# NTV-UIT/MARLLB

Measured on AMD Instinct MI355X. Metric: env-steps/sec (whole node), 4-server LB env, batch 4k→512k at 1/2/4/8 MI355X, higher is better.
Workload: dtype fp32/int32 (f64 reward); 1 GPU; LB env random-policy rollout, 4 servers (BASELINE configs[1] rollout at the north-star batch); assign_policy=sed, envs_per_gpu=65536, servers=4, global_batch=65536, autoreset=True, autoreset_mode=same_step, parallelism=env-shard x1, dyn_mapping=auto

## Files before the change

### marllb_amd/csrc/lbsim_api.hip

```cpp
#include <hip/hip_runtime.h>

#include <cxxabi.h>

#include <algorithm>
#include <cmath>
#include <cstdarg>
#include <cstdio>
#include <cstdlib>
#include <cstring>
#include <string>
#include <vector>

#include "../../include/lbsim.h"
#include "lbsim_internal.h"
#include "lbsim_fused.h"
#include "lbsim_nets.h"
#include "lbsim_stateless.h"
#include "lbsim_vpp.h"

using namespace lbk;

namespace {
constexpr int kLogMax = 8;
thread_local const void* g_log_fn[kLogMax];
// ... 450 lines not shown
    for (int i = 0; i < g_log_n; ++i) v.emplace_back(g_log_cls[i], g_log_fn[i]);
    h->launched_lost[which] = g_log_lost;
    g_log_n = 0;
    g_log_lost = 0;
    g_log_class = -1;
  }
};

std::string short_kernel_name(const char* raw) {
  std::string s = raw ? raw : "?";
  int st = 0;
  if (char* d = abi::__cxa_demangle(s.c_str(), nullptr, nullptr, &st)) {
    if (st == 0) s = d;
    free(d);
  }
  int depth = 0;
  for (size_t i = 0; i < s.size(); ++i) {
    if (s[i] == '<') ++depth;
    else if (s[i] == '>') --depth;
    else if (s[i] == '(' && depth == 0 && s.compare(i, 21, "(anonymous namespace)") != 0) {
      s.resize(i);
      break;
    }
  }
  for (const char* pre : {"void ", "lbk::", "(anonymous namespace)::"}) {
    for (size_t at; (at = s.find(pre)) != std::string::npos;) s.erase(at, strlen(pre));
  }
  return s;
}

LaunchCtx ctx(const lbsim_t* h) { return LaunchCtx{h->plan, h->st, h->prm, h->flow}; }

StepPlan plan_of(const lbsim_t* h) {
  static const Overrides ov = Overrides::from_env();
  const SimParams& p = h->prm;
  PlanInput in{};
  in.B = h->B, in.S = h->S, in.Q = p.Q, in.policy = p.policy;
  in.trace = p.trace != 0, in.fail = p.fail_thr != 0u, in.leak = p.leak != 0;
  in.split = p.split != 0, in.res_vpp = p.res_vpp != 0, in.dur_plane = dur_plane(p);
  in.next_reset = p.next_reset != 0;
  in.flow_stats = h->flow.hist != nullptr;
  in.dyn_mapping = h->cfg.dyn_mapping, in.step_kernel = h->cfg.step_kernel, in.simds = h->simds;
  return make_plan(in, ov);
}

int launch_dynamics(lbsim_t* h, const void* action, int dtype, int32_t* assign,
                    const uint8_t* mask, int mode, hipStream_t stream) {
  ProfScope ps(h, stream, mode == kModeStep ? 0 : 2);
  if (mode == kModeStep && h->plan.nr)
    launch_dynamics_step_nr(ctx(h), action, dtype, assign, mask, stream);
  else if (mode == kModeStep)
    launch_dynamics_step(ctx(h), action, dtype, assign, mask, stream);
  else
    launch_dynamics_reset(ctx(h), action, dtype, assign, mask, stream);
  return launch_check(h, "dynamics_kernel");
}

bool facade_bad(const lbsim_t* h, const lbsim_step_outputs_t* out) {
  if (out->agent_obs == nullptr && out->state == nullptr) return false;
  return out->num_agents < 1 || out->servers_per_agent < 1 ||
         (int64_t)out->num_agents * out->servers_per_agent != h->S;
}

ObsOutputs obs_outputs(const lbsim_step_outputs_t* out, bool reset) {
  ObsOutputs o{};
  o.obs = out->obs;
  o.raw_obs = out->raw_obs;
  if (!reset) {
    o.reward = out->reward;
    o.done = out->done;
    o.ep_len = out->episode_length;
    o.ep_ret = out->episode_return;
    o.done_word = out->done_word;
    o.done_value = out->done_value;
  }
  o.agent_obs = out->agent_obs;
  o.state = out->state;
  o.num_agents = out->num_agents;
  o.servers_per_agent = out->servers_per_agent;
  return o;
}

int launch_observe(lbsim_t* h, const ObsOutputs& o, const uint8_t* mask, int mode,
                   hipStream_t stream) {
  ProfScope ps(h, stream, mode == kModeStep ? 1 : 3);
  if (mode == kModeStep) launch_observe_step(ctx(h), o, mask, stream);
  else launch_observe_reset(ctx(h), o, mask, stream);
  return launch_check(h, "observe_kernel");
}


int round16(int x) { return (x + 15) / 16 * 16; }

int fused_mt(int dflt) {
  static const int forced = env_int("LBSIM_FUSED_MT", 0);
  return (forced == 1 || forced == 2 || forced == 4) ? forced : dflt;
}

}

extern "C" {

const char* lbsim_version(void) { return "lbsim 0.1.0 (gfx950, HIP)"; }
int lbsim_abi_version(void) { return LBSIM_ABI_VERSION; }

int lbsim_config_default(lbsim_config_t* c) {
  if (c == nullptr) return LBSIM_EINVAL;
  memset(c, 0, sizeof(*c));
  c->num_envs = 1;
  c->num_servers = 4;
  c->env_id_offset = 0;
  c->seed = 0;
  c->action_type = LBSIM_ACTION_DISCRETE;
  c->num_discrete = 3;
  c->discrete_weights[0] = 1.0f;
  c->discrete_weights[1] = 1.5f;
  c->discrete_weights[2] = 2.0f;
  c->min_weight = 0.1f;
  c->max_weight = 10.0f;
  c->reward_metric = LBSIM_METRIC_JAIN;
  c->reward_field = 10;
  c->step_interval = 0.25f;
  c->max_steps = 10000;
  c->normalize_obs = 0;
  c->assign_policy = LBSIM_POLICY_SED;
  c->arrival_source = LBSIM_ARRIVAL_POISSON;
  c->arrival_rate = 400.0f;
  for (int s = 0; s < LBSIM_MAX_SERVERS; ++s) c->server_rate[s] = 125.0f;
  c->decay_factor = 0.9f;
  c->queue_capacity = 32;
  c->warmup_steps = 8;
  c->lost_fin_prob = 0.0f;
  c->flow_timeout_s = 40.0f;
  c->flow_buckets = 1024;
  c->fail_prob = 0.0f;
  c->recover_prob = 0.1f;
  c->duration_mode = LBSIM_DURATION_AGE;
  c->lost_fin_pending = 256;
  c->reservoir_mode = LBSIM_RESERVOIR_ALGR;
  return LBSIM_OK;
}

int lbsim_config_validate(const lbsim_config_t* cfg, char* msg, size_t msg_len) {
  return validate(cfg, msg, msg_len);
}

int lbsim_create(const lbsim_config_t* cfg, int device, lbsim_t** out) {
  if (out == nullptr) return fail(nullptr, LBSIM_EINVAL, "out is NULL");
  *out = nullptr;
  char msg[256] = {0};
  if (validate(cfg, msg, sizeof(msg)) != LBSIM_OK) return fail(nullptr, LBSIM_EINVAL, "%s", msg);
  int ndev = 0;
  if (hipGetDeviceCount(&ndev) != hipSuccess || ndev == 0)
    return fail(nullptr, LBSIM_EDEVICE, "no HIP device available");
  if (device < 0 || device >= ndev)
    return fail(nullptr, LBSIM_EINVAL, "device %d out of range [0, %d)", device, ndev);
  DeviceGuard g(device);
  if (!g.ok) return fail(nullptr, LBSIM_EDEVICE, "hipSetDevice(%d) failed", device);

  lbsim_t* h = new lbsim_t();
  h->cfg = *cfg;
  h->device = device;
  int cus = 0;
  if (hipDeviceGetAttribute(&cus, hipDeviceAttributeMultiprocessorCount, device) != hipSuccess ||
      cus < 1)
    cus = 256;
  h->simds = 4 * cus;
  h->B = cfg->num_envs;
  h->S = cfg->num_servers;
  h->Q = cfg->queue_capacity;
  h->initialised = false;
  memset(&h->st, 0, sizeof(h->st));
  derive_params(*cfg, h->prm);
  h->plan = plan_of(h);
  for (Section& sec : sections(h)) {
    void* p = nullptr;
    if (hipMalloc(&p, sec.bytes) != hipSuccess) {
      lbsim_destroy(h);
      return fail(nullptr, LBSIM_ENOMEM, "hipMalloc(%zu) failed", sec.bytes);
    }
    h->allocs.push_back(p);
    *sec.ptr = p;
    if (hipMemset(p, 0, sec.bytes) != hipSuccess) {
      lbsim_destroy(h);
      return fail(nullptr, LBSIM_EDEVICE, "hipMemset failed");
    }
  }
  if (cfg->normalize_obs) {
    const size_t n = (size_t)h->B * h->S * NF;
    hipLaunchKernelGGL(init_norm_std, dim3((unsigned)((n + 255) / 256)), dim3(256), 0, nullptr,
                       h->st.norm_std, n);
  }
  if (hipDeviceSynchronize() != hipSuccess) {
    lbsim_destroy(h);
    return fail(nullptr, LBSIM_EDEVICE, "device init failed");
  }
  *out = h;
  return LBSIM_OK;
}

int lbsim_destroy(lbsim_t* h) {
  if (h == nullptr) return LBSIM_OK;
  {
    DeviceGuard g(h->device);
    for (void* p : h->allocs) (void)hipFree(p);
    if (h->trace_buf) (void)hipFree(h->trace_buf);
    if (h->stats_buf) (void)hipFree(h->stats_buf);
    if (h->rates_buf) (void)hipFree(h->rates_buf);
    if (h->flow_buf) (void)hipFree(h->flow_buf);
    for (hipEvent_t e : h->prof.ev) (void)hipEventDestroy(e);
  }
  delete h;
  return LBSIM_OK;
}

const char* lbsim_last_error(const lbsim_t* h) {
  return h ? h->err.c_str() : g_create_err.c_str();
}

int lbsim_dynamics_kernel(const lbsim_t* h) {
  if (h == nullptr) return -1;
  return h->plan.dyn.kernel;
}

int lbsim_seed(lbsim_t* h, uint64_t seed) {
  if (h == nullptr) return LBSIM_EINVAL;
  DeviceGuard g(h->device);
  h->cfg.seed = seed;
  h->prm.key0 = (uint32_t)(seed & 0xFFFFFFFFull);
  h->prm.key1 = (uint32_t)(seed >> 32);
  if (hipMemset(h->st.episode, 0, (size_t)h->B * 4) != hipSuccess)
    return fail(h, LBSIM_EDEVICE, "hipMemset failed");
  return LBSIM_OK;
}

int lbsim_reset(lbsim_t* h, const uint8_t* env_mask, float* obs_out, void* stream) {
  lbsim_step_outputs_t o;
  memset(&o, 0, sizeof(o));
  o.obs = obs_out;
  return lbsim_reset_ex(h, env_mask, &o, stream);
}

int lbsim_reset_ex(lbsim_t* h, const uint8_t* env_mask, const lbsim_step_outputs_t* out,
                   void* stream) {
  if (h == nullptr) return LBSIM_EINVAL;
  if (out == nullptr || out->obs == nullptr) return fail(h, LBSIM_EINVAL, "obs_out is NULL");
  if (facade_bad(h, out)) return fail(h, LBSIM_EINVAL, "agent_obs / state need num_agents * "
                                                       "servers_per_agent == num_servers");
  if (h->prm.trace && h->prm.trace_rows == 0)
    return fail(h, LBSIM_EINVAL, "arrival_source TRACE: call lbsim_set_trace before lbsim_reset");
  DeviceGuard g(h->device);
  LaunchLog log(h, 1);
  const hipStream_t s = (hipStream_t)stream;
  h->reset_seen = true;
  int rc = launch_dynamics(h, nullptr, 0, nullptr, env_mask, kModeReset, s);
  if (rc != LBSIM_OK) return rc;
  const ObsOutputs o = obs_outputs(out, true);
  rc = launch_observe(h, o, env_mask, kModeReset, s);
  if (rc != LBSIM_OK) return rc;
  if (env_mask == nullptr) h->initialised = true;
  return LBSIM_OK;
}

int lbsim_step(lbsim_t* h, const void* action, int action_dtype, float* obs_out,
               float* reward_out, uint8_t* done_out, int32_t* assign_count_out, void* stream) {
  lbsim_step_outputs_t o;
  memset(&o, 0, sizeof(o));
  o.obs = obs_out;
  o.reward = reward_out;
  o.done = done_out;
  o.assign_count = assign_count_out;
  return lbsim_step_ex(h, action, action_dtype, &o, stream);
}

size_t lbsim_config_size(void) { return sizeof(lbsim_config_t); }
size_t lbsim_step_outputs_size(void) { return sizeof(lbsim_step_outputs_t); }

int lbsim_step_ex(lbsim_t* h, const void* action, int action_dtype,
                  const lbsim_step_outputs_t* out, void* stream) {
  if (h == nullptr) return LBSIM_EINVAL;
  if (!h->initialised) return fail(h, LBSIM_EINVAL, "call lbsim_reset before lbsim_step");
  if (out == nullptr || action == nullptr || out->obs == nullptr || out->reward == nullptr ||
      out->done == nullptr)
    return fail(h, LBSIM_EINVAL, "action/obs/reward/done buffers must be non-NULL");
  if (h->cfg.action_type == LBSIM_ACTION_DISCRETE) {
    if (action_dtype != LBSIM_DTYPE_I32 && action_dtype != LBSIM_DTYPE_I64)
      return fail(h, LBSIM_EINVAL, "discrete actions must be int32 or int64");
  } else if (action_dtype != LBSIM_DTYPE_F32) {
    return fail(h, LBSIM_EINVAL, "continuous actions must be float32");
  }
  if (facade_bad(h, out)) return fail(h, LBSIM_EINVAL, "agent_obs / state need num_agents * "
                                                       "servers_per_agent == num_servers");
  if (out->done_word != nullptr && h->B != 1)
    return fail(h, LBSIM_EINVAL, "done_word needs a one-env handle (num_envs = 1)");
  DeviceGuard g(h->device);
  LaunchLog log(h, 0);
  const hipStream_t s = (hipStream_t)stream;
  const ObsOutputs o = obs_outputs(out, false);
  if (h->plan.form == kStepWave) {
    ProfScope ps(h, s, 4);
    launch_step_wave(ctx(h), action, action_dtype, out->assign_count, o, s);
    return launch_check(h, "step_wave_kernel");
  }
  if (h->plan.form == kStepGroupFused) {
    ProfScope ps(h, s, 4);
    launch_fused_step(ctx(h), action, action_dtype, out->assign_count, o, s);
    return launch_check(h, "fused_step_kernel");
  }
  h->prof.chain = true;
  int rc = launch_dynamics(h, action, action_dtype, out->assign_count, nullptr, kModeStep, s);
  h->prof.chain = false;
  if (rc != LBSIM_OK) {
    h->prof.chain_ev = -1;
    return rc;
  }
  return launch_observe(h, o, nullptr, kModeStep, s);
}

int lbsim_step_stats(lbsim_t* h, int64_t* stats_out) {
  if (h == nullptr || stats_out == nullptr) return LBSIM_EINVAL;
  DeviceGuard g(h->device);
  if (h->stats_buf == nullptr && hipMalloc(&h->stats_buf, 16) != hipSuccess) {
    h->stats_buf = nullptr;
    return fail(h, LBSIM_ENOMEM, "hipMalloc(16) failed");
  }
  const int64_t n = (int64_t)h->B * h->S;
  unsigned long long host[2] = {0, 0};
  if (hipDeviceSynchronize() != hipSuccess || hipMemset(h->stats_buf, 0, 16) != hipSuccess)
    return fail(h, LBSIM_EDEVICE, "sync / memset failed");
  const int64_t blocks = std::min<int64_t>((n + 255) / 256, 4096);
  hipLaunchKernelGGL(step_stats_kernel, dim3((unsigned)blocks), dim3(256), 0, nullptr, h->st.chg,
                     h->st.hc, n, h->stats_buf);
  if (hipMemcpy(host, h->stats_buf, 16, hipMemcpyDeviceToHost) != hipSuccess)
    return fail(h, LBSIM_EDEVICE, "step_stats_kernel failed");
  stats_out[0] = (int64_t)host[0];
  stats_out[1] = (int64_t)host[1];
  return LBSIM_OK;
}

int lbsim_episode_stats(lbsim_t* h, int32_t* length_out, double* return_out, void* stream) {
  if (h == nullptr) return LBSIM_EINVAL;
  DeviceGuard g(h->device);
  hipLaunchKernelGGL(copy_episode_stats, dim3((unsigned)((h->B + 255) / 256)), dim3(256), 0,
                     (hipStream_t)stream, h->st.ep_step, h->st.ep_return, length_out, return_out,
                     h->B);
  return launch_check(h, "copy_episode_stats");
}

int lbsim_reward(const lbsim_config_t* cfg, const float* obs, int64_t n, float* reward_out,
                 void* stream) {
  if (cfg == nullptr || obs == nullptr || reward_out == nullptr || n < 0) return LBSIM_EINVAL;
  if (cfg->num_servers < 1 || cfg->num_servers > LBSIM_MAX_SERVERS) return LBSIM_EINVAL;
  if (cfg->reward_metric < 0 || cfg->reward_metric > 8) return LBSIM_EINVAL;
  if (n == 0) return LBSIM_OK;
  hipLaunchKernelGGL(reward_kernel, dim3((unsigned)((n + 255) / 256)), dim3(256), 0,
                     (hipStream_t)stream, obs, n, cfg->num_servers, cfg->reward_metric,
                     cfg->reward_field, reward_out);
  return hipGetLastError() == hipSuccess ? LBSIM_OK : LBSIM_EDEVICE;
}

int lbsim_set_trace(lbsim_t* h, const uint32_t* gap_us, const float* work, int64_t rows,
                    void* stream) {
  if (h == nullptr) return LBSIM_EINVAL;
  if (!h->prm.trace) return fail(h, LBSIM_EINVAL, "lbsim_set_trace needs arrival_source TRACE");
  if (gap_us == nullptr || work == nullptr || rows < 1 || rows > (int64_t)0x7FFFFFFF)
    return fail(h, LBSIM_EINVAL, "trace: need device gap_us/work and 1 <= rows < 2^31");
  DeviceGuard g(h->device);
  const hipStream_t s = (hipStream_t)stream;
  if (hipStreamSynchronize(s) != hipSuccess) return fail(h, LBSIM_EDEVICE, "stream sync failed");
  if (h->trace_buf) {
    (void)hipFree(h->trace_buf);
    h->trace_buf = nullptr;
    h->prm.trace_rows = 0;
  }
  const size_t n = (size_t)rows;
  if (hipMalloc(&h->trace_buf, n * 8) != hipSuccess) {
    h->trace_buf = nullptr;
    return fail(h, LBSIM_ENOMEM, "hipMalloc(%zu) failed", n * 8);
  }
  uint32_t* g_dev = (uint32_t*)h->trace_buf;
  float* w_dev = (float*)(g_dev + n);
  if (hipMemcpyAsync(g_dev, gap_us, n * 4, hipMemcpyDeviceToDevice, s) != hipSuccess ||
      hipMemcpyAsync(w_dev, work, n * 4, hipMemcpyDeviceToDevice, s) != hipSuccess ||
      hipStreamSynchronize(s) != hipSuccess)
    return fail(h, LBSIM_EDEVICE, "trace copy failed");
  h->st.trace_gap = g_dev;
  h->st.trace_work = w_dev;
  h->prm.trace_rows = (uint32_t)rows;
  return LBSIM_OK;
}

int lbsim_set_env_rates(lbsim_t* h, const float* arrival_rate, const float* server_rate,
                        void* stream) {
  if (h == nullptr) return LBSIM_EINVAL;
  if (arrival_rate != nullptr && h->prm.lf_thr != 0u)
    return fail(h, LBSIM_ENOTSUP, "per-env arrival rates on a lost-FIN handle (lost_fin_prob > 0): "
                                  "the bucket-wait mean and the 32-bit guess bound depend on the "
                                  "arrival rate (per-env server rates are allowed)");
  if (arrival_rate != nullptr && h->prm.trace)
    return fail(h, LBSIM_ENOTSUP, "per-env arrival rates on a TRACE handle: the trace sets the "
                                  "arrival rate (per-env server rates are allowed)");
  if (arrival_rate == nullptr && server_rate == nullptr) return LBSIM_OK;
  DeviceGuard g(h->device);
  const hipStream_t s = (hipStream_t)stream;
  int rc = env_rates_ensure(h, s);
  if (rc != LBSIM_OK) return rc;
  const size_t B = (size_t)h->B, BS = B * h->S;
  const EnvRates live = env_rates_live(h), stg = env_rates_staging(h);
  uint32_t* const bad = env_rates_bad(h);
  if (hipMemsetAsync(bad, 0, sizeof(uint32_t), s) != hipSuccess)
    return fail(h, LBSIM_EDEVICE, "per-env rates: hipMemsetAsync failed");
  hipLaunchKernelGGL(env_rates_kernel, dim3((unsigned)((BS + 255) / 256)), dim3(256), 0, s,
                     arrival_rate, (int64_t)1, server_rate, (int64_t)h->S, h->B, h->S, stg, bad);
  rc = launch_check(h, "env_rates_kernel");
  if (rc != LBSIM_OK) return rc;
  uint32_t nbad = 0;
  if (hipMemcpyAsync(&nbad, bad, sizeof(nbad), hipMemcpyDeviceToHost, s) != hipSuccess ||
      hipStreamSynchronize(s) != hipSuccess)
    return fail(h, LBSIM_EDEVICE, "per-env rates: conversion failed");
  if (nbad != 0u)
    return fail(h, LBSIM_EINVAL, "per-env rates: %u value(s) out of range (arrival_rate must be in "
                                 "[0.1, 1e6] flows/s, server_rate in [1, 1e7]; NaN rejected)", nbad);
  bool ok = true;
  if (arrival_rate != nullptr) {
    ok &= hipMemcpyAsync(live.arrival, stg.arrival, B * 4, hipMemcpyDeviceToDevice, s) == hipSuccess;
    ok &= hipMemcpyAsync(live.gap, stg.gap, B * 4, hipMemcpyDeviceToDevice, s) == hipSuccess;
  }
  if (server_rate != nullptr) {
    ok &= hipMemcpyAsync(live.server, stg.server, BS * 4, hipMemcpyDeviceToDevice, s) == hipSuccess;
    ok &= hipMemcpyAsync(live.scale, stg.scale, BS * 4, hipMemcpyDeviceToDevice, s) == hipSuccess;
  }
  if (!ok) return fail(h, LBSIM_EDEVICE, "per-env rates: device copy failed");
  h->st.env_gap = live.gap;
  h->st.env_scale = live.scale;
  return LBSIM_OK;
}

int lbsim_clear_env_rates(lbsim_t* h) {
  if (h == nullptr) return LBSIM_EINVAL;
  h->st.env_gap = nullptr;
  h->st.env_scale = nullptr;
  if (h->rates_buf == nullptr) return LBSIM_OK;
  DeviceGuard g(h->device);
  if (hipDeviceSynchronize() != hipSuccess) return fail(h, LBSIM_EDEVICE, "sync failed");
  env_rates_fill_defaults(h, nullptr);
  const int rc = launch_check(h, "env_rates_kernel");
  if (rc != LBSIM_OK) return rc;
  if (hipDeviceSynchronize() != hipSuccess) return fail(h, LBSIM_EDEVICE, "sync failed");
  return LBSIM_OK;
}

int lbsim_get_env_rates(lbsim_t* h, float* arrival_rate_out, float* server_rate_out,
                        void* stream) {
  if (h == nullptr) return LBSIM_EINVAL;
  if (arrival_rate_out == nullptr && server_rate_out == nullptr) return LBSIM_OK;
  DeviceGuard g(h->device);
  const hipStream_t s = (hipStream_t)stream;
  const int rc = env_rates_ensure(h, s);
  if (rc != LBSIM_OK) return rc;
  const size_t B = (size_t)h->B, BS = B * h->S;
  const EnvRates live = env_rates_live(h);
  bool ok = true;
  if (arrival_rate_out != nullptr)
    ok &= hipMemcpyAsync(arrival_rate_out, live.arrival, B * 4, hipMemcpyDeviceToDevice, s) == hipSuccess;
  if (server_rate_out != nullptr)
    ok &= hipMemcpyAsync(server_rate_out, live.server, BS * 4, hipMemcpyDeviceToDevice, s) == hipSuccess;
  return ok ? LBSIM_OK : fail(h, LBSIM_EDEVICE, "per-env rates: device copy failed");
}

int lbsim_flow_stats_enable(lbsim_t* h) {
  if (h == nullptr) return LBSIM_EINVAL;
  if (h->flow_buf != nullptr) return LBSIM_OK;
  if (h->reset_seen)
    return fail(h, LBSIM_EINVAL, "lbsim_flow_stats_enable must precede the handle's first "
                                 "lbsim_reset (the statistics change which kernels it launches)");
  DeviceGuard g(h->device);
  const size_t BS = (size_t)h->B * h->S, bytes = flow_stats_bytes(BS);
  void* p = nullptr;
  if (hipMalloc(&p, bytes) != hipSuccess) return fail(h, LBSIM_ENOMEM, "hipMalloc(%zu) failed", bytes);
  if (hipMemset(p, 0, bytes) != hipSuccess || hipDeviceSynchronize() != hipSuccess) {
    (void)hipFree(p);
    return fail(h, LBSIM_EDEVICE, "flow statistics: hipMemset failed");
  }
  h->flow_buf = p;
  h->flow.sum = (unsigned long long*)p;
  h->flow.hist = (uint32_t*)(h->flow.sum + BS);
  h->flow.count = h->flow.hist + BS * kFlowBins;
  h->flow.max_us = h->flow.count + BS;
  h->plan = plan_of(h);
  return LBSIM_OK;
}

int lbsim_flow_stats_get(lbsim_t* h, uint32_t* count, uint64_t* sum_us, uint32_t* max_us,
                         uint32_t* hist, void* stream) {
  if (h == nullptr) return LBSIM_EINVAL;
  if (h->flow_buf == nullptr)
    return fail(h, LBSIM_ENOTSUP, "flow statistics are off: call lbsim_flow_stats_enable first");
  DeviceGuard g(h->device);
  const hipStream_t s = (hipStream_t)stream;
  const size_t BS = (size_t)h->B * h->S;
  const FlowStats& f = h->flow;
  bool ok = true;
  if (count != nullptr)
    ok &= hipMemcpyAsync(count, f.count, BS * 4, hipMemcpyDeviceToDevice, s) == hipSuccess;
  if (sum_us != nullptr)
    ok &= hipMemcpyAsync(sum_us, f.sum, BS * 8, hipMemcpyDeviceToDevice, s) == hipSuccess;
  if (max_us != nullptr)
    ok &= hipMemcpyAsync(max_us, f.max_us, BS * 4, hipMemcpyDeviceToDevice, s) == hipSuccess;
  if (hist != nullptr)
    ok &= hipMemcpyAsync(hist, f.hist, BS * kFlowBins * 4, hipMemcpyDeviceToDevice, s) ==
          hipSuccess;
  return ok ? LBSIM_OK : fail(h, LBSIM_EDEVICE, "flow statistics: device copy failed");
}

int lbsim_flow_stats_quantiles(lbsim_t* h, const uint32_t* q_ppm, int nq, int per_server,
                               uint32_t* out_us, void* stream) {
  if (h == nullptr) return LBSIM_EINVAL;
  if (h->flow_buf == nullptr)
    return fail(h, LBSIM_ENOTSUP, "flow statistics are off: call lbsim_flow_stats_enable first");
  if (q_ppm == nullptr || out_us == nullptr || nq < 1 || nq > 16)
    return fail(h, LBSIM_EINVAL, "flow quantiles: need device q_ppm / out_us and 1 <= nq <= 16 "
                                 "(got %d)", nq);
  DeviceGuard g(h->device);
  const size_t rows = per_server ? (size_t)h->B * h->S : (size_t)h->B;
  hipLaunchKernelGGL(flow_quantiles_kernel, dim3((unsigned)rows), dim3(64), 0, (hipStream_t)stream,
                     h->flow.hist, h->flow.max_us, q_ppm, nq, h->S, per_server ? 1 : 0, out_us);
  return launch_check(h, "flow_quantiles_kernel");
}

int lbsim_flow_stats_clear(lbsim_t* h, const uint8_t* env_mask, void* stream) {
  if (h == nullptr) return LBSIM_EINVAL;
  if (h->flow_buf == nullptr)
    return fail(h, LBSIM_ENOTSUP, "flow statistics are off: call lbsim_flow_stats_enable first");
  DeviceGuard g(h->device);
  const int64_t n = (int64_t)h->B * h->S * kFlowBins;
  hipLaunchKernelGGL(flow_clear_kernel, dim3((unsigned)((n + 255) / 256)), dim3(256), 0,
                     (hipStream_t)stream, h->flow.count, h->flow.sum, h->flow.max_us,
                     h->flow.hist, n, h->S, env_mask);
  return launch_check(h, "flow_clear_kernel");
}

int lbsim_agent_obs(const float* obs, int64_t n, int S, int num_agents, int servers_per_agent,
                    float* out, void* stream) {
  if (n < 0 || S < 1 || S > LBSIM_MAX_SERVERS || num_agents < 1 || servers_per_agent < 1 ||
      num_agents * servers_per_agent != S)
    return LBSIM_EINVAL;
  if (n == 0) return LBSIM_OK;
  if (!obs || !out) return LBSIM_EINVAL;
  const int64_t total = n * num_agents * (4 * servers_per_agent + 7 * S);
  hipLaunchKernelGGL(agent_obs_kernel, dim3((unsigned)((total + 255) / 256)), dim3(256), 0,
                     (hipStream_t)stream, obs, n, S, num_agents, servers_per_agent, out);
  return hipGetLastError() == hipSuccess ? LBSIM_OK : LBSIM_EDEVICE;
}

int lbsim_gru_gates(const float* gi, const float* gh, const float* h, float* h_out, int64_t B,
                    int H, void* stream) {
  if (B < 0 || H < 1 || (B > 0 && (!gi || !gh || !h || !h_out))) return LBSIM_EINVAL;
  if (B == 0) return LBSIM_OK;
  const int64_t n = B * H;
  hipLaunchKernelGGL(gru_gates_kernel, dim3((unsigned)((n + 255) / 256)), dim3(256), 0,
                     (hipStream_t)stream, gi, gh, h, h_out, B, H);
  return hipGetLastError() == hipSuccess ? LBSIM_OK : LBSIM_EDEVICE;
}

int lbsim_sac_head(const float* y, int64_t B, int A, float log_std_min, float log_std_max,
                   float action_scale, float action_bias, int deterministic, uint64_t seed,
                   uint32_t step, float* action_out, float* log_std_out, void* stream) {
  if (B < 0 || A < 1 || (B > 0 && (!y || !action_out))) return LBSIM_EINVAL;
  if (B == 0) return LBSIM_OK;
  const int64_t n = B * A;
  hipLaunchKernelGGL(sac_head_kernel, dim3((unsigned)((n + 255) / 256)), dim3(256), 0,
                     (hipStream_t)stream, y, B, A, log_std_min, log_std_max, action_scale,
                     action_bias, deterministic, (uint32_t)(seed & 0xFFFFFFFFull),
                     (uint32_t)(seed >> 32), step, action_out, log_std_out);
  return hipGetLastError() == hipSuccess ? LBSIM_OK : LBSIM_EDEVICE;
}

int lbsim_qmix_tail(const float* q, const float* w1, int64_t w1_ld, const float* b1,
                    int64_t b1_ld, const float* w2, int64_t w2_ld, const float* b2, int64_t b2_ld,
                    int64_t B, int A, int E, float* q_tot, void* stream) {
  if (B < 0 || A < 1 || E < 1) return LBSIM_EINVAL;
  if (B == 0) return LBSIM_OK;
  if (!q || !w1 || !b1 || !w2 || !b2 || !q_tot) return LBSIM_EINVAL;
  hipLaunchKernelGGL(qmix_tail_kernel, dim3((unsigned)((B + 255) / 256)), dim3(256), 0,
                     (hipStream_t)stream, q, w1, w1_ld, b1, b1_ld, w2, w2_ld, b2, b2_ld, B, A, E,
                     q_tot);
  return hipGetLastError() == hipSuccess ? LBSIM_OK : LBSIM_EDEVICE;
}

size_t lbsim_sac_actor_size(void) { return sizeof(lbsim_sac_actor_t); }
size_t lbsim_qmix_policy_size(void) { return sizeof(lbsim_qmix_policy_t); }

int lbsim_sac_actor_step(const lbsim_sac_actor_t* n, const float* state, float* hidden,
                         const uint8_t* reset_mask, int64_t B, int deterministic, uint64_t seed,
                         uint32_t step, float* action_out, float* log_std_out, void* stream) {
  if (n == nullptr || B < 0 || n->state_dim < 1 || n->state_dim > 512 || n->action_dim < 1 ||
      n->action_dim > 16)
    return LBSIM_EINVAL;
  if (n->gru_dim != 128 || n->hidden_dim != 256) return LBSIM_ENOTSUP;
  if (B == 0) return LBSIM_OK;
  if (!state || !hidden || !action_out || !n->w_ih || !n->w_hh || !n->b_ih || !n->b_hh ||
      !n->w1 || !n->b1 || !n->wh || !n->bh)
    return LBSIM_EINVAL;
  SacActorArgs a{};
  a.state = state;
  a.hidden = hidden;
  a.reset = reset_mask;
// ... 283 lines not shown
```

### marllb_amd/csrc/lbsim_plan.h

```cpp
#pragma once
#include <cstdint>
#include <cstdlib>
#include <cstring>

#include "../../include/lbsim.h"

namespace lbk {

struct Overrides {
  bool group_lanes_set = false;
  int group_lanes = 0;
  int dyn_wave = -1;
  int dyn_epw = 0;
  int step_kernel = LBSIM_STEP_AUTO;
  int step_wave_occ = 0;

  static Overrides from_env() {
    const auto num = [](const char* name, int dflt) {
      const char* e = std::getenv(name);
      return e ? std::atoi(e) : dflt;
    };
    Overrides o;
    o.group_lanes_set = std::getenv("LBSIM_DYN_GROUP_LANES") != nullptr;
    o.group_lanes = num("LBSIM_DYN_GROUP_LANES", 0);
    o.dyn_wave = num("LBSIM_DYN_WAVE", -1);
    o.dyn_epw = num("LBSIM_DYN_EPW", 0);
    const char* k = std::getenv("LBSIM_STEP_KERNEL");
    if (k != nullptr && std::strcmp(k, "split") == 0) o.step_kernel = LBSIM_STEP_SPLIT;
    if (k != nullptr && std::strcmp(k, "fused") == 0) o.step_kernel = LBSIM_STEP_FUSED;
    o.step_wave_occ = num("LBSIM_STEP_WAVE_OCC", 0);
    return o;
  }
};

struct PlanInput {
  int B, S, Q;
  int policy;
  bool trace;
  bool fail;
  bool leak;
  bool split;
  bool res_vpp;
  bool dur_plane;
  bool next_reset;
  int dyn_mapping;
  int step_kernel;
  int simds;
  bool flow_stats;
};

enum StepForm { kStepWave, kStepGroupFused, kStepTwoLaunch };
enum ObsForm { kObsPair, kObsPair16, kObsPairChunks, kObsSplit, kObsReset8, kObsChunked };

constexpr int kObsChunkServers = 4;
constexpr int kObsScratchBytes = 7840;
constexpr int kObsReset8Envs = 8;
constexpr int kObserveSplitS = 16;
constexpr unsigned env_lane_block(int maxs) { return maxs <= 8 ? 256u : 128u; }

struct DynPlan {
  int kernel;
  int width;
  bool full;
  int waves;
  int epw;
  unsigned grid, block;
};

struct ObsPlan {
  int form;
  int maxs;
  int nchunks;
  unsigned chunk_grid;
  unsigned grid, block, lds;
};

struct StepPlan {
  int form;
  int width;
  int occ;
  int obs_maxs;
  unsigned grid;
  bool nr;
  DynPlan dyn, reset_dyn;
  ObsPlan obs, reset_obs;
};

inline StepPlan make_plan(const PlanInput& in, const Overrides& ov) {
  const int S = in.S;
  const int64_t B = in.B, simds = in.simds;
  const auto blocks = [](int64_t n, int64_t per) { return (unsigned)((n + per - 1) / per); };
  StepPlan p{};

  const bool full_only = in.res_vpp || in.flow_stats;
  const bool wave_fits = ov.dyn_wave != 0 && !ov.group_lanes_set &&
                         in.dyn_mapping != LBSIM_DYN_ENV_PER_LANE && S <= 8 && in.Q <= 32 &&
                         in.policy != LBSIM_POLICY_ALIAS && !in.fail && !in.leak && !in.split &&
                         !full_only;
  const bool wave_ok = wave_fits && (ov.dyn_wave == 1 || B <= (S <= 4 ? 4 : 2) * simds);
  const int ng = S <= 2 ? 1 : S <= 4 ? 2 : 4;

  const int fl = ov.group_lanes;
  int g = 8;
  if (in.dyn_mapping == LBSIM_DYN_ENV_PER_LANE && S <= 16 && !in.split && !full_only) g = 0;
  else if (fl >= S && (fl == 4 || fl == 8 || fl == 16 || fl == 32 || fl == 64)) g = fl;
  else if (S <= 2) g = 2;
  else if (S <= 4) g = B * 4 / 64 <= in.simds / 2 ? 8 : 4;
  else while (g < S) g <<= 1;
  const bool full = in.leak || in.dur_plane || full_only;

  const auto dynamics = [&](bool step) {
    DynPlan d{};
    if (wave_ok) {
      d = {LBSIM_DYN_KERNEL_WAVE, ng, false, 0, 0, (unsigned)B, 64u};
    } else if (g == 0) {
      const int maxs = S <= 4 ? 4 : S <= 8 ? 8 : 16;
      d = {LBSIM_DYN_KERNEL_ENV_LANE, maxs, false, 0, 0, blocks(B, env_lane_block(maxs)),
           env_lane_block(maxs)};
    } else {
      const int epw = ov.dyn_epw >= 1 && ov.dyn_epw <= 64 / g ? ov.dyn_epw : 64 / g;
      d = {LBSIM_DYN_KERNEL_GROUP, g, full, 1, epw, blocks(B, epw), 64u};
      if (full) d.waves = 0;
      else if (step && in.next_reset) d.waves = 4;
      else if (step && in.policy == LBSIM_POLICY_SED && (g == 4 || g == 8) && d.grid > 4 * simds)
        d.waves = 5;
    }
    return d;
  };
  p.dyn = dynamics(true);
  p.reset_dyn = dynamics(false);
  p.nr = in.next_reset;

  const int k = in.step_kernel != LBSIM_STEP_AUTO ? in.step_kernel : ov.step_kernel;
  p.form = kStepTwoLaunch;
  if (wave_fits && !in.next_reset &&
      (k == LBSIM_STEP_FUSED ? wave_ok : k == LBSIM_STEP_AUTO && B <= 4 * simds)) {
    p.form = kStepWave;
    p.width = ng;
    const bool occ2 = ov.step_wave_occ == 2 || (ov.step_wave_occ != 4 && B <= 2 * simds);
    p.occ = occ2 ? 2 : 4;
    p.obs_maxs = ng == 4 ? 8 : kObsChunkServers;
    p.grid = (unsigned)B;
  } else if (k == LBSIM_STEP_FUSED && !in.next_reset && !full && g >= 2 && g <= 16) {
    p.form = kStepGroupFused;
    p.width = g;
    p.obs_maxs = g < 4 ? 4 : g;
    p.grid = blocks(B, 64 / g);
  }

  const int nw = (S + kObsChunkServers - 1) / kObsChunkServers;
  const auto observe = [&](bool step) {
    ObsPlan o{};
    if (step && !in.dur_plane && (S <= 8 || S % 8 == 0)) {
      if (S <= 8) o = {kObsPair, 0, 0, 0u, blocks(B, 8 / S), 64u, 0u};
      else if (S == 16) o = {kObsPair16, 0, 0, 0u, (unsigned)B, 128u, 0u};
      else o = {kObsPairChunks, 64, S / 8, (unsigned)(B * (S / 8)), (unsigned)B, 64u, 0u};
    } else if (S > kObsChunkServers && S > kObserveSplitS) {
      o = {kObsSplit, S <= 8 ? 8 : S <= 16 ? 16 : 64, nw, (unsigned)(B * nw), (unsigned)B, 64u, 0u};
    } else if (!step && S <= kObsChunkServers) {
      o = {kObsReset8, 0, 0, 0u, blocks(B, kObsReset8Envs), 64u * kObsReset8Envs,
           (unsigned)(kObsReset8Envs * kObsScratchBytes)};
    } else {
      o = {kObsChunked, S <= 4 ? 4 : S <= 8 ? 8 : S <= 16 ? 16 : 64, nw, 0u, (unsigned)B,
           64u * nw, (unsigned)(nw * kObsScratchBytes)};
    }
    return o;
  };
  p.obs = observe(true);
  p.reset_obs = observe(false);
  return p;
}

}
```

### marllb_amd/csrc/lbsim_step.hip

```cpp
#include "lbsim_internal.h"
#include "lbsim_dyn_group.h"
#include "lbsim_dyn_wave.h"


namespace lbk {
namespace {

template <int G, int MAXS, int POLICY, bool TRACE>
__global__ void __launch_bounds__(64)
    fused_step_kernel(DevState st, SimParams p, const void* action, int action_dtype,
                      int32_t* assign_out, ObsOutputs out) {
  __shared__ union {
    DynGroupLds<POLICY> dyn;
    ObsScratch obs;
  } L;
  __shared__ float s_obs[MAXS * NF];
  __shared__ float s_act[MAXS];
  const int lane = (int)threadIdx.x;
  dyn_group_wave<G, kModeStep, POLICY, TRACE>(st, p, action, action_dtype, assign_out, nullptr,
                                              blockIdx.x, lane, L.dyn);
  __syncthreads();
  constexpr int EPW = 64 / G;
  for (int i = 0; i < EPW; ++i) {
    const size_t b = (size_t)blockIdx.x * EPW + (size_t)i;
    if (b >= (size_t)p.B) break;
    observe_env_wave<MAXS>(st, p, out, b, L.obs, s_obs, s_act, lane);
  }
}

template <int NG, int POLICY, bool TRACE, int OCC, int MAXS = kObsChunk>
__global__ void __launch_bounds__(64, OCC)
    step_wave_kernel(DevState st, SimParams p, const void* action, int action_dtype,
                     int32_t* assign_out, ObsOutputs out) {
  __shared__ union {
    WaveLds dyn;
    ObsScratch obs;
  } L;
  __shared__ float s_obs[MAXS * NF];
  __shared__ float s_act[MAXS];
  const int lane = (int)threadIdx.x;
  if (!dyn_wave_env<NG, kModeStep, POLICY, TRACE, OCC == 2>(st, p, action, action_dtype,
                                                            assign_out, nullptr, blockIdx.x, lane,
                                                            L.dyn))
    return;
  __syncthreads();
  observe_env_wave<MAXS>(st, p, out, blockIdx.x, L.obs, s_obs, s_act, lane);
}

}

void launch_step_wave(const LaunchCtx& L, const void* action, int dtype, int32_t* assign,
                      const ObsOutputs& o, hipStream_t s) {
  const StepPlan& p = L.plan;
  pick<1, 2, 4>(p.width, [&](auto N) { pick<0, 1, 2, 3>(L.prm.policy, [&](auto P) {
    pick_bool(L.prm.trace != 0, [&](auto T) { pick<2, 4>(p.occ, [&](auto OCC) {
      constexpr int NG = decltype(N)::value;
      LBSIM_LAUNCH((step_wave_kernel<NG, decltype(P)::value, decltype(T)::value,
                                     decltype(OCC)::value, (NG == 4 ? 8 : kObsChunk)>),
                   dim3(p.grid), dim3(64), 0, s, L.st, L.prm, action, dtype, assign, o);
    }); });
  }); });
}

void launch_fused_step(const LaunchCtx& L, const void* action, int dtype, int32_t* assign,
                       const ObsOutputs& o, hipStream_t s) {
  const StepPlan& p = L.plan;
  pick<2, 4, 8, 16>(p.width, [&](auto GG) { pick<0, 1, 2, 3, 4>(L.prm.policy, [&](auto P) {
    pick_bool(L.prm.trace != 0, [&](auto T) {
      constexpr int G = decltype(GG)::value;
      LBSIM_LAUNCH((fused_step_kernel<G, (G < 4 ? 4 : G), decltype(P)::value, decltype(T)::value>),
                   dim3(p.grid), dim3(64), 0, s, L.st, L.prm, action, dtype, assign, o);
    });
  }); });
}

}
```

Measured before the change: 289.1 million env-steps/s.

## Fuse group dynamics and paired observe into one step kernel at mid-size batches

Adds a fuse_pair plan flag. It routes the default two-launch step (group dynamics followed by the paired observe kernel) into a single fused_step_kernel when the dynamics grid spans roughly 2–4 waves per SIMD. The fused kernel gains a PAIR path that runs observe_rows_paired and observe_outputs per env group inside the same block after dynamics. It reloads state and params from the kernarg segment to hold down register pressure, and it sets occupancy through launch bounds. The aim is to remove a kernel launch and the inter-kernel gap, and to reread freshly written state while it may still be cached. The cost is that observe now runs with the dynamics kernel's block mapping and occupancy.

```diff
diff --git a/marllb_amd/csrc/lbsim_api.hip b/marllb_amd/csrc/lbsim_api.hip
--- a/marllb_amd/csrc/lbsim_api.hip
+++ b/marllb_amd/csrc/lbsim_api.hip
@@ -776,7 +776,7 @@
     launch_step_wave(ctx(h), action, action_dtype, out->assign_count, o, s);
     return launch_check(h, "step_wave_kernel");
   }
-  if (h->plan.form == kStepGroupFused) {
+  if (h->plan.form == kStepGroupFused || h->plan.fuse_pair) {
     ProfScope ps(h, s, 4);
     launch_fused_step(ctx(h), action, action_dtype, out->assign_count, o, s);
     return launch_check(h, "fused_step_kernel");
diff --git a/marllb_amd/csrc/lbsim_plan.h b/marllb_amd/csrc/lbsim_plan.h
--- a/marllb_amd/csrc/lbsim_plan.h
+++ b/marllb_amd/csrc/lbsim_plan.h
@@ -84,7 +84,11 @@
   bool nr;
   DynPlan dyn, reset_dyn;
   ObsPlan obs, reset_obs;
+  bool fuse_pair;
 };
+
+constexpr int kFusePairMinWaves = 2;
+constexpr int kFusePairMaxWaves = 4;
 
 inline StepPlan make_plan(const PlanInput& in, const Overrides& ov) {
   const int S = in.S;
@@ -168,6 +172,11 @@
   };
   p.obs = observe(true);
   p.reset_obs = observe(false);
+
+  p.fuse_pair = k == LBSIM_STEP_AUTO && p.form == kStepTwoLaunch && !in.next_reset &&
+                p.dyn.kernel == LBSIM_DYN_KERNEL_GROUP && !p.dyn.full && g <= 16 &&
+                p.dyn.epw == 64 / g && p.obs.form == kObsPair &&
+                p.dyn.grid >= kFusePairMinWaves * simds && p.dyn.grid <= kFusePairMaxWaves * simds;
   return p;
 }
 
diff --git a/marllb_amd/csrc/lbsim_step.hip b/marllb_amd/csrc/lbsim_step.hip
--- a/marllb_amd/csrc/lbsim_step.hip
+++ b/marllb_amd/csrc/lbsim_step.hip
@@ -1,30 +1,66 @@
+#include <cstddef>
+
 #include "lbsim_internal.h"
 #include "lbsim_dyn_group.h"
 #include "lbsim_dyn_wave.h"
 
-
 namespace lbk {
 namespace {
 
-template <int G, int MAXS, int POLICY, bool TRACE>
-__global__ void __launch_bounds__(64)
+struct FusedStepArgs {
+  DevState st;
+  SimParams p;
+  const void* action;
+  int action_dtype;
+  int32_t* assign_out;
+  ObsOutputs out;
+};
+
+template <int G, int MAXS, int POLICY, bool TRACE, bool PAIR, bool FAC>
+__global__ void __launch_bounds__(64, PAIR ? kObsPairWaves : 1)
     fused_step_kernel(DevState st, SimParams p, const void* action, int action_dtype,
                       int32_t* assign_out, ObsOutputs out) {
   __shared__ union {
     DynGroupLds<POLICY> dyn;
     ObsScratch obs;
   } L;
-  __shared__ float s_obs[MAXS * NF];
-  __shared__ float s_act[MAXS];
+  __shared__ float s_obs[(PAIR ? 8 : MAXS) * NF];
+  __shared__ float s_act[PAIR ? 8 : MAXS];
   const int lane = (int)threadIdx.x;
   dyn_group_wave<G, kModeStep, POLICY, TRACE>(st, p, action, action_dtype, assign_out, nullptr,
                                               blockIdx.x, lane, L.dyn);
   __syncthreads();
   constexpr int EPW = 64 / G;
-  for (int i = 0; i < EPW; ++i) {
-    const size_t b = (size_t)blockIdx.x * EPW + (size_t)i;
-    if (b >= (size_t)p.B) break;
-    observe_env_wave<MAXS>(st, p, out, b, L.obs, s_obs, s_act, lane);
+  if constexpr (PAIR) {
+    typedef const char __attribute__((address_space(4))) * KernArgs;
+    KernArgs ka = (KernArgs)__builtin_amdgcn_kernarg_segment_ptr();
+    int ln = lane;
+    int epu = 1;
+#pragma clang loop unroll(disable)
+    for (int e0 = 0; e0 < EPW; e0 += epu) {
+      asm volatile("" : "+s"(ka), "+v"(ln));
+      const DevState& st2 = *(const DevState*)(ka + offsetof(FusedStepArgs, st));
+      const SimParams& p2 = *(const SimParams*)(ka + offsetof(FusedStepArgs, p));
+      const ObsOutputs& out2 = *(const ObsOutputs*)(ka + offsetof(FusedStepArgs, out));
+      const int S = p2.S;
+      epu = 8 / S;
+      const size_t B = (size_t)p2.B, b0 = (size_t)blockIdx.x * EPW + (size_t)e0;
+      if (b0 >= B) break;
+      int nenv = EPW - e0 < epu ? EPW - e0 : epu;
+      nenv = B - b0 < (size_t)nenv ? (int)(B - b0) : nenv;
+      observe_rows_paired<true>(st2, p2, b0, nenv, L.obs, s_obs, ln);
+      for (int e = 0; e < nenv; ++e) {
+        observe_outputs<8, kModeStep, FAC>(st2, p2, out2, b0 + (size_t)e, s_obs + e * S * NF,
+                                           s_act, ln, 64);
+        wave_sync();
+      }
+    }
+  } else {
+    for (int i = 0; i < EPW; ++i) {
+      const size_t b = (size_t)blockIdx.x * EPW + (size_t)i;
+      if (b >= (size_t)p.B) break;
+      observe_env_wave<MAXS>(st, p, out, b, L.obs, s_obs, s_act, lane);
+    }
   }
 }
 
@@ -65,12 +101,23 @@
 void launch_fused_step(const LaunchCtx& L, const void* action, int dtype, int32_t* assign,
                        const ObsOutputs& o, hipStream_t s) {
   const StepPlan& p = L.plan;
-  pick<2, 4, 8, 16>(p.width, [&](auto GG) { pick<0, 1, 2, 3, 4>(L.prm.policy, [&](auto P) {
-    pick_bool(L.prm.trace != 0, [&](auto T) {
+  const bool own = p.form == kStepGroupFused;
+  const int width = own ? p.width : p.dyn.width;
+  const dim3 grid(own ? p.grid : p.dyn.grid);
+  const bool pair = p.obs.form == kObsPair;
+  const bool fac = !pair || o.agent_obs != nullptr || o.state != nullptr;
+  pick<2, 4, 8, 16>(width, [&](auto GG) { pick<0, 1, 2, 3, 4>(L.prm.policy, [&](auto P) {
+    pick_bool(L.prm.trace != 0, [&](auto T) { pick_bool(pair, [&](auto PR) {
       constexpr int G = decltype(GG)::value;
-      LBSIM_LAUNCH((fused_step_kernel<G, (G < 4 ? 4 : G), decltype(P)::value, decltype(T)::value>),
-                   dim3(p.grid), dim3(64), 0, s, L.st, L.prm, action, dtype, assign, o);
-    });
+      constexpr bool PAIR = decltype(PR)::value;
+      const auto launch = [&](auto F) {
+        LBSIM_LAUNCH((fused_step_kernel<G, (G < 4 ? 4 : G), decltype(P)::value, decltype(T)::value,
+                                        PAIR, decltype(F)::value>),
+                     grid, dim3(64), 0, s, L.st, L.prm, action, dtype, assign, o);
+      };
+      if constexpr (PAIR) pick_bool(fac, launch);
+      else launch(std::true_type{});
+    }); });
   }); });
 }
 
```

Measured after the change: 285.2 million env-steps/s. 1.3% lower.
